# wjqkkky/TTS

Measured on AMD Instinct MI355X. Metric: mel-frames/s (Tacotron2-DDC + MB-MelGAN end-to-end), higher is better.
Workload: dtype f32; 1 GPU; C2: Tacotron2-DDC (r_init=7, r=2, sigmoid attn) + MB-MelGAN [8,4,2]x4, 32 LJ-length utterances per GPU; global_batch=32, r=2, parallelism=replicas x1

## Files before the change

### tts_amd/csrc/api_core.hip

```cpp
#include "host.h"
#include "split16.h"
#include "switches.h"

#include <cmath>
#include <cstring>
#include <memory>

static thread_local std::string g_err;
void tts_set_error(const std::string& m) { g_err = m; }

namespace ttsh {

void upload_split_rows(DevBuf& d, const std::vector<float>& w, int rows, int K) {
  bool ok = rows % 16 == 0 && K % 32 == 0 && w.size() == (size_t)rows * K;
  for (float v : w) ok &= std::fabs(v) < F16_RANGE;
  if (!ok) {
    d.reset();
    return;
  }
  d.upload(pack_split_a(rows / 16, K / 32, [&](int m, int k) { return w[(size_t)m * K + k]; }));
}

const HostT& need(const HostMap& m, const std::string& k, std::vector<int64_t> shape) {
  auto it = m.find(k);
// ... 116 lines not shown
  a.rep_pad = c.rep_pad;
  a.nphase = L.nphase;
  for (int i = 0; i < 8; ++i) a.pad_left[i] = L.pad_left[i];
  a.w_phase_stride = L.phase_stride;
  a.W = L.W.f();
  a.bias = L.bias.f();
  a.Cout = L.Cout;
  a.Cout_pad = L.Cout_pad;
  a.out = c.out;
  a.ob = c.ob;
  a.oc = c.oc;
  a.ot = c.ot;
  a.out_mul = c.out_mul;
  a.epi_act = c.epi;
  a.resid = c.resid;
  a.rb = c.rb;
  a.rc = c.rc;
  a.rt = c.rt;
  a.resid_rows = c.resid_rows;
  a.aux = c.aux;
  a.auxb = c.auxb;
  a.max_q = c.max_q;
  a.B = c.B;
  a.merged_u = c.merged_u;
  TTS_CHECK(!c.merged_u || (c.oflow && L.W16.p), "phase-merged ConvTranspose runs on split-f16 weights only");
  if (c.oflow && L.W16.p && c.nsrc == 1 && (c.s[0].sc != 1 || c.s[0].st % 4 == 0)) {
    a.W16 = L.W16.p;
    a.w16_phase_stride = L.w16_stride;
    a.oflow = c.oflow;
    launch_conv_x3(a, st);
    return;
  }
  launch_conv(a, L.tile, st);
}

void enter(tts_ctx* c, void* stream) {
  if (c->sv_live && !c->in_submit) {
    HIP_OK(hipStreamWaitEvent(c->s, c->ev_sv, 0));
    c->sv_live = false;
  }
  if (hipStreamQuery((hipStream_t)stream) == hipSuccess) return;
  (void)hipGetLastError();
  HIP_OK(hipEventRecord(c->ev_in, (hipStream_t)stream));
  HIP_OK(hipStreamWaitEvent(c->s, c->ev_in, 0));
}
void leave(tts_ctx* c, void* stream) {
// ... 150 lines not shown
```

### tts_amd/csrc/api_ge2e.hip

```cpp
#include "host.h"
#include "gsync.h"
#include "split16.h"
#include "switches.h"

#include <cmath>

using namespace ttsh;

namespace {

__global__ void pad_channels_kernel(const float* __restrict__ x, int D, int Dp, long n_rows, float* __restrict__ y) {
  for (long i = (long)blockIdx.x * blockDim.x + threadIdx.x; i < n_rows * Dp; i += (long)gridDim.x * blockDim.x) {
    const long r = i / Dp;
    const int c = (int)(i - r * Dp);
    y[i] = c < D ? x[r * D + c] : 0.f;
  }
}

__global__ __launch_bounds__(256) void ge2e_final_kernel(const float* __restrict__ src, long sb, int width,
                                                         const int* lens, int T_max, const float* __restrict__ W,
                                                         const float* __restrict__ bias, int P,
                                                         float* __restrict__ out) {
  __shared__ float v[1024], red[4];
  const int b = blockIdx.x, tid = threadIdx.x;
// ... 110 lines not shown
  TTS_CHECK(T_max >= 1 && T_max <= 100000, "speaker encoder: bad T_max");
  for (int b = 0; b < B; ++b) TTS_CHECK(h_lens[b] >= 1 && h_lens[b] <= T_max, "speaker encoder: lens out of range");
  hipStream_t s = c->s;
  const int H = G.H;
  long gen = 0;
  grow<float>(W.x, (size_t)B * T_max * G.in_pad, gen);
  grow<int>(W.lens, 64, gen);
  grow<float>(W.g, (size_t)B * T_max * 4 * H, gen);
  grow<float>(W.o, (size_t)B * T_max * H, gen);
  grow<float>(W.p, (size_t)B * T_max * G.proj, gen);
  grow<unsigned>(W.bar, BAR_WORDS, gen);
  grow<float>(W.hbuf, (size_t)2 * 64 * H, gen);
  std::vector<int> lens(h_lens, h_lens + B);
  HIP_OK(hipMemcpyAsync(W.lens.p, lens.data(), B * 4, hipMemcpyHostToDevice, s));
  pad_channels_kernel<<<1024, 256, 0, s>>>(d_x, G.in_dim, G.in_pad, (long)B * T_max, W.x.f());
  HIP_OK(hipGetLastError());
  const float* in = W.x.f();
  int din = G.in_pad;
  const bool pipe_env = sw::ge2e_pipe();
  bool piped = false;
  if (pipe_env && c->gemm_x3 && G.pipe_ok && B <= 16) {
    ConvCall cc;
    cc.lens = W.lens.i();
    cc.B = B;
    cc.oflow = x3_flag(c);
    cc.max_q = T_max;
    cc.s[0] = src_of(in, (long)T_max * din, 1, din, din, 0);
    cc.out = W.g.f();
    cc.ob = (long)T_max * 4 * H;
    cc.oc = 1;
    cc.ot = 4 * H;
    run_conv(G.gin[0], cc, s);
    const uint16_t* w16[4] = {nullptr, nullptr, nullptr, nullptr};
    const float* bias[4] = {nullptr, nullptr, nullptr, nullptr};
    for (int l = 0; l < G.nl; ++l) {
      w16[l] = l == 0 ? G.whh16[0].h() : G.wpipe[l].h();
      bias[l] = l == 0 ? nullptr : G.bpipe[l].f();
    }
    piped = launch_ge2e_pipe(w16, bias, G.nl, W.g.f(), W.lens.i(), T_max, B, W.hbuf.f(),
                             reinterpret_cast<unsigned*>(W.bar.p), W.o.f(), s);
    if (piped && G.with_proj) {
      ConvCall cp;
      cp.lens = W.lens.i();
      cp.B = B;
      cp.oflow = x3_flag(c);
      cp.max_q = T_max;
      cp.s[0] = src_of(W.o.f(), (long)T_max * H, 1, H, H, 0);
      cp.out = W.p.f();
      cp.ob = (long)T_max * G.proj;
      cp.oc = 1;
      cp.ot = G.proj;
      run_conv(G.proj_l[G.nl - 1], cp, s);
    }
  }
  for (int l = 0; l < G.nl && !piped; ++l) {
    ConvCall cc;
    cc.lens = W.lens.i();
    cc.B = B;
    cc.oflow = x3_flag(c);
    cc.max_q = T_max;
    cc.s[0] = src_of(in, (long)T_max * din, 1, din, din, 0);
    cc.out = W.g.f();
    cc.ob = (long)T_max * 4 * H;
    cc.oc = 1;
    cc.ot = 4 * H;
    run_conv(G.gin[l], cc, s);
    const bool ok = launch_lstm768_persist(W.g.f(), G.whh[l].f(), c->gemm_x3 ? G.whh16[l].h() : nullptr, W.lens.i(),
                                           T_max, B, W.hbuf.f(),
                                           reinterpret_cast<unsigned*>(W.bar.p), W.o.f(), s);
    TTS_CHECK(ok, "speaker encoder: cooperative launch unavailable");
    if (G.with_proj) {
      ConvCall cp;
      cp.lens = W.lens.i();
      cp.B = B;
      cp.oflow = x3_flag(c);
      cp.max_q = T_max;
      cp.s[0] = src_of(W.o.f(), (long)T_max * H, 1, H, H, 0);
      cp.out = W.p.f();
      cp.ob = (long)T_max * G.proj;
      cp.oc = 1;
      cp.ot = G.proj;
      run_conv(G.proj_l[l], cp, s);
      in = W.p.f();
      din = G.proj;
    } else {
      in = W.o.f();
      din = H;
    }
  }
  if (G.with_proj)
    ge2e_final_kernel<<<B, 256, 0, s>>>(W.p.f(), (long)T_max * G.proj, G.proj, W.lens.i(), T_max, nullptr, nullptr,
                                        G.proj, d_out);
  else
    ge2e_final_kernel<<<B, 256, 0, s>>>(W.o.f(), (long)T_max * H, H, W.lens.i(), T_max, G.lin_w.f(), G.lin_b.f(),
                                        G.proj, d_out);
  HIP_OK(hipGetLastError());
// ... 32 lines not shown
```

### tts_amd/csrc/api_glow.hip

```cpp
#include "host.h"

#include <cmath>
#include <cstdlib>

using namespace ttsh;

namespace {

std::pair<std::vector<float>, std::vector<float>> interleave_halves(const std::vector<float>& w,
                                                                           const std::vector<float>& b, int half,
                                                                           int rowlen) {
  std::vector<float> wo(w.size()), bo(b.size());
  for (int r = 0; r < 2 * half; ++r) {
    const int src = (r & 1) ? half + r / 2 : r / 2;
    std::copy(w.begin() + (size_t)src * rowlen, w.begin() + (size_t)(src + 1) * rowlen, wo.begin() + (size_t)r * rowlen);
    bo[r] = b[src];
  }
  return {wo, bo};
}

void glow_finalize(tts_ctx* c, int num_chars, int enc_layers, int flows, int wn_layers) {
  auto& G = c->glow;
  const auto& h = c->glow_host;
  G.ready = false;
// ... 275 lines not shown
    }
    W.h_spk.assign(h_spk, h_spk + B);
    HIP_OK(hipMemcpyAsync(W.spk.p, W.h_spk.data(), B * 4, hipMemcpyHostToDevice, s));
    launch_glow_speaker(W.spk.i(), G.emb_g.f(), G.c_in, G.c_pad, W.g.f(), B, s);
    ConvCall cc;
    cc.lens = W.ones.i();
    cc.B = B;
    cc.oflow = x3_flag(c);
    cc.max_q = 1;
    cc.s[0] = src_of(W.g.f(), G.c_pad, 1, 1, G.c_pad, 0);
    cc.out = W.gcond.f();
    cc.ob = NC;
    cc.oc = 1;
    cc.ot = 1;
    run_conv(G.cond, cc, s);
  }
  float* x = W.xa.f();
  float* x2 = W.xb.f();
  launch_glow_embed(d_ids, T, G.emb.f(), G.num_chars, H, dl, x, B, s);
  auto conv = [&](const ConvLayer& L, const float* in, int cin, float* out, int cout, int epi,
                  const float* resid = nullptr) {
    ConvCall cc;
    cc.lens = dl;
    cc.B = B;
    cc.oflow = x3_flag(c);
    cc.max_q = T;
    cc.s[0] = src_of(in, (long)cin * T, T, 1, cin, 0);
    cc.out = out;
    cc.ob = (long)cout * T;
    cc.oc = T;
    cc.ot = 1;
    cc.epi = epi;
    cc.resid = resid;
    cc.rb = (long)cout * T;
    cc.rc = T;
    cc.rt = 1;
    run_conv(L, cc, s);
  };
  if (G.tdsep || G.tfm) {
    float* h0 = W.h2.f();
    float* h1 = W.hdp.f();
    conv(G.pre_conv[0], x, H, h0, H, 0);
    launch_ln(h0, (long)H * T, H, G.pre_g[0].f(), G.pre_b[0].f(), dl, B, T, s, true);
    conv(G.pre_conv[1], h0, H, h1, H, 0);
    launch_ln(h1, (long)H * T, H, G.pre_g[1].f(), G.pre_b[1].f(), dl, B, T, s, true);
    conv(G.pre_conv[2], h1, H, h0, H, 0);
// ... 7 lines not shown
      conv(G.tfm_o[i], h0, H, x2, H, 0, x);
      launch_ln(x2, (long)H * T, H, G.tfm_g1[i].f(), G.tfm_b1[i].f(), dl, B, T, s);
      conv(G.tfm_f1[i], x2, H, big, 768, 1);
      conv(G.tfm_f2[i], big, 768, x, H, 0, x2);
      launch_ln(x, (long)H * T, H, G.tfm_g2[i].f(), G.tfm_b2[i].f(), dl, B, T, s);
    }
    for (int i = 0; i < (G.tdsep ? G.enc_layers : 0); ++i) {
      conv(G.tds_tc[i], x, H, h0, H, 6);
      launch_tds_depthwise(h0, H, T, G.tds_dw[i].f(), G.tds_dwb[i].f(), dl, h1, B, s);
      conv(G.tds_tc2[i], h1, H, x2, H, 0, x);
      std::swap(x, x2);
    }
  }
  for (int i = 0; i < (G.tdsep || G.tfm ? 0 : G.enc_layers); ++i) {
    conv(G.enc_conv[i], x, H, W.h2.f(), 2 * H, 0);
    launch_glu_ln_res(W.h2.f(), (long)2 * H * T, 2 * H, G.enc_g[i].f(), G.enc_b[i].f(), x, (long)H * T, x2,
                      (long)H * T, dl, B, T, s);
    std::swap(x, x2);
  }
  conv(G.proj_m, x, H, W.om.f(), C, 0);
  if (G.c_pad > 0) {
    ConvCall cc;
    cc.lens = dl;
    cc.B = B;
    cc.max_q = T;
    cc.nsrc = 2;
    cc.s[0] = src_of(x, (long)H * T, T, 1, H, 0);
    cc.s[1] = src_of(W.g.f(), G.c_pad, 1, 0, G.c_pad, 0);
    cc.out = W.hdp.f();
    cc.ob = (long)F * T;
    cc.oc = T;
    cc.ot = 1;
    cc.epi = 1;
    run_conv(G.dp1, cc, s);
  } else {
    conv(G.dp1, x, H, W.hdp.f(), F, 1);
  }
  launch_ln(W.hdp.f(), (long)F * T, F, G.dp_g1.f(), G.dp_b1.f(), dl, B, T, s);
  conv(G.dp2, W.hdp.f(), F, W.h2.f(), F, 1);
  launch_ln(W.h2.f(), (long)F * T, F, G.dp_g2.f(), G.dp_b2.f(), dl, B, T, s);
  conv(G.dp_proj, W.h2.f(), F, W.logw.f(), 1, 0);
  launch_glow_durations(W.logw.f(), T, dl, length_scale, W.cum.f(), W.ylens.i(), W.wceil.f(), B, s);
  HIP_OK(hipMemcpyAsync(h_ylens, W.ylens.p, B * 4, hipMemcpyDeviceToHost, s));
  HIP_OK(hipStreamSynchronize(s));
  int mx = 1;
  W.h_ylens.assign(h_ylens, h_ylens + B);
// ... 9 lines not shown
  TTS_CHECK(W.B > 0 && Ty == W.Ty, "glow: decode after encode with Ty = max(y_lengths)");
  hipStream_t s = c->s;
  const int B = W.B, Tx = W.Tx, H = G.H, C = G.C, C2 = 2 * C, K = Ty / 2;
  long gen = 0;
  const int K1 = std::max(K, 1);
  grow<float>(W.z, (size_t)B * C * Ty, gen);
  grow<float>(W.sq, (size_t)B * C2 * K1, gen);
  grow<float>(W.sq2, (size_t)B * C2 * K1, gen);
  grow<float>(W.whs, (size_t)B * 2 * H * K1, gen);
  grow<float>(W.wacts, (size_t)B * H * K1, gen);
  launch_glow_expand(W.om.f(), C, Tx, W.lens.i(), W.cum.f(), W.ylens.i(), Ty, d_noise, noise_scale, d_ymean, W.z.f(),
                     d_attn, B, s);
  HIP_OK(hipMemcpyAsync(d_logw, W.logw.p, (size_t)B * Tx * 4, hipMemcpyDeviceToDevice, s));
  HIP_OK(hipMemsetAsync(d_y, 0, (size_t)B * C * 2 * K * 4, s));
  if (K == 0) return;
  for (int b = 0; b < B; ++b) W.h_klens[b] = W.h_ylens[b] / 2;
  HIP_OK(hipMemcpyAsync(W.klens.p, W.h_klens.data(), B * 4, hipMemcpyHostToDevice, s));
  const int* kl = W.klens.i();
  launch_glow_squeeze(W.z.f(), C, Ty, W.ylens.i(), W.sq.f(), K, B, s);
  auto conv = [&](const ConvLayer& L, const float* in, int in_rows, float* out, int out_rows, const float* resid,
                  int epi, int resid_rows = 0, const float* aux = nullptr) {
    ConvCall cc;
    cc.lens = kl;
    cc.B = B;
    cc.oflow = x3_flag(c);
    cc.max_q = K;
    cc.s[0] = src_of(in, (long)in_rows * K, K, 1, L.Cin, 0);
    cc.out = out;
    cc.ob = (long)out_rows * K;
    cc.oc = K;
    cc.ot = 1;
    cc.resid = resid;
    cc.rb = (long)out_rows * K;
    cc.rc = K;
    cc.rt = 1;
    cc.epi = epi;
    cc.resid_rows = resid_rows;
    cc.aux = aux;
    cc.auxb = (long)G.flows * G.wn_layers * 2 * H;
    run_conv(L, cc, s);
  };
  float* x = W.sq.f();
  float* x2 = W.sq2.f();
  float* hid = W.whs.f();
  float* skip = W.whs.f() + (size_t)H * K;
  for (int k = G.flows - 1; k >= 0; --k) {
// ... 53 lines not shown
```

### tts_amd/csrc/api_melgan.hip

```cpp
#include "host.h"
#include "split16.h"
#include "switches.h"

#include <cmath>
#include <cstring>

using namespace ttsh;

static void melgan_finalize(tts_ctx* c, int in_ch, int out_ch, int base, const int32_t* ups, int n_up, int nres,
                     int use_pqmf) {
  auto& G = c->mg;
  const auto& m = c->mg_host;
  G.ready = false;
  TTS_CHECK(nres >= 1 && nres <= 4, "num_res_blocks must be in [1, 4] (dilation <= 27)");
  G.in_ch = in_ch;
  G.out_ch = out_ch;
  G.base = base;
  G.nres = nres;
  G.pqmf = use_pqmf;
  G.ups.assign(ups, ups + n_up);
  G.convT.clear();
  G.dconv.clear();
  G.fused.clear();
  G.convT.resize(n_up);
// ... 123 lines not shown
  int up = 1;
  for (int u : G.ups) up *= u;
  size_t maxelems = (size_t)G.base * Lb;
  {
    int mul = 1, Cc = G.base;
    for (int u : G.ups) {
      mul *= u;
      Cc /= 2;
      maxelems = std::max(maxelems, (size_t)Cc * Lb * mul);
    }
  }
  int* vld = c->vlens_override;
  if (!vld) {
    W.lens.ensure(B * 4);
    vld = W.lens.i();
  }
  W.xa.ensure((size_t)B * maxelems * 4);
  W.xb.ensure((size_t)B * maxelems * 4);
  std::vector<int> lens(h_lens, h_lens + B);
  if (!dev_lens) HIP_OK(hipMemcpyAsync(vld, lens.data(), B * 4, hipMemcpyHostToDevice, s));
  else TTS_CHECK(c->vlens_override || W.lens.bytes >= (size_t)B * 4, "vocoder lengths buffer");
  ConvCall cc;
  cc.lens = vld;
  cc.B = B;
  cc.oflow = x3_flag(c);
  cc.len_add = 2 * pad;
  if (mel_strides) {
    TTS_CHECK(mel_strides[1] >= 1 && mel_strides[2] >= 1 && mel_strides[1] < (1L << 31) && mel_strides[2] < (1L << 31) &&
                  (mel_strides[0] >= 1 || B == 1) && mel_strides[0] >= 0,
              "mel strides must be positive");
    TTS_CHECK(mel_strides[1] != 1 || (mel_strides[2] % 4 == 0 && (reinterpret_cast<uintptr_t>(mel) & 15) == 0),
              "channel stride 1 needs a frame stride divisible by 4 and a 16-byte aligned mel");
    cc.s[0] = src_of(mel, (long)mel_strides[0], (int)mel_strides[1], (int)mel_strides[2], G.in_ch, 0);
  } else {
    cc.s[0] = src_of(mel, (long)G.in_ch * M_max, M_max, 1, G.in_ch, 0);
  }
  cc.pad_mode = 1;
  cc.rep_pad = pad;
  cc.in_mul = cc.q_mul = 1;
  cc.max_q = Lb;
  float* x = W.xa.f();
  float* xo = W.xb.f();
  int C = G.base, mul = 1;
  long Ls = Lb;
  cc.out = x;
  cc.ob = (long)C * Ls;
// ... 241 lines not shown
```

### tts_amd/csrc/api_taco.hip

```cpp
#include "host.h"
#include "decoder.h"
#include "gsync.h"
#include "split16.h"
#include "switches.h"

#include <cstdio>
#include <cstring>

using namespace ttsh;

namespace {

DecDev make_dev(tts_ctx* c, int Bact) {
  auto& W = c->tws;
  DecDev d{};
  int* ci = W.ctl.i();
  d.ctl = reinterpret_cast<DecCtl*>(ci);
  d.done = ci + 4;
  d.steps = ci + 4 + BMAX;
  d.status = ci + 4 + 2 * BMAX;
  d.max_steps = ci + 4 + 3 * BMAX;
  d.lens = W.lens.i();
  d.dec_out = W.dec.f();
  d.align_out = W.align.f();
// ... 165 lines not shown
  for (int m = 0; m < MB; ++m) acc[m] = 0.f;
  for (int e = q; e < Es; e += 4) {
    const float w = WT[(long)e * N + nc];
#pragma unroll
    for (int m = 0; m < MB; ++m) {
      const float sv = m < B ? spk[m * Es + e] : 0.f;
      acc[m] = fmaf(sv, w, acc[m]);
    }
  }
  if (q > 0) {
#pragma unroll
    for (int m = 0; m < MB; ++m) red[q - 1][m][c] = acc[m];
  }
  __syncthreads();
  if (q != 0 || n >= N) return;
  const float base = n >= pj0 ? pjb[n - pj0] : 0.f;
#pragma unroll
  for (int m = 0; m < MB; ++m)
    if (m < Bp) out[(long)m * N + n] = base + (m < B ? ((acc[m] + red[0][m][c]) + red[1][m][c]) + red[2][m][c] : 0.f);
  for (int m = MB; m < Bp; ++m) out[(long)m * N + n] = base;
}

void run_encoder(tts_ctx* c, const int64_t* ids, int B, int T_max, float* enc_out, hipStream_t s,
                 const int* rowmap = nullptr) {
  auto& M = c->taco;
  auto& W = c->tws;
  const int* lens = W.lens.i();
  launch_embed_gather(ids, T_max, M.emb.f(), M.num_chars, 512, lens, B, W.x0.f(), s, rowmap);
  ConvCall cc;
  cc.lens = lens;
  cc.B = B;
  cc.oflow = x3_flag(c);
  cc.max_q = T_max;
  cc.pad_mode = 0;
  cc.epi = 1;
  cc.s[0] = src_of(W.x0.f(), (long)T_max * 512, 1, 512, 512, 0);
  cc.out = W.ca.f();
  cc.ob = (long)512 * T_max;
  cc.oc = T_max;
  cc.ot = 1;
  run_conv(M.enc[0], cc, s);
  cc.s[0] = src_of(W.ca.f(), (long)512 * T_max, T_max, 1, 512, 0);
  cc.out = W.cb.f();
  run_conv(M.enc[1], cc, s);
  cc.s[0] = src_of(W.cb.f(), (long)512 * T_max, T_max, 1, 512, 0);
  cc.out = W.ca.f();
  run_conv(M.enc[2], cc, s);
  cc.s[0] = src_of(W.ca.f(), (long)512 * T_max, T_max, 1, 512, 0);
  cc.out = W.gin.f();
  cc.ob = (long)2048 * T_max;
  cc.oc = 1;
  cc.ot = 2048;
  cc.epi = 0;
  run_conv(M.lstm_in, cc, s);
  W.enc_ndom = sw::encoder_steps()
                   ? 0
                   : launch_bilstm_persist(W.gin.f(), M.whhT.f(), c->gemm_x3 ? M.whhT16.h() : nullptr, lens, T_max, B,
                                           W.lh.f(), reinterpret_cast<unsigned*>(W.lc.p), enc_out, s);
  W.enc_persist = W.enc_ndom > 0;
  if (!W.enc_persist) {
    HIP_OK(hipMemsetAsync(enc_out, 0, (size_t)B * T_max * 512 * 4, s));
    launch_bilstm(W.gin.f(), M.whhT.f(), lens, T_max, B, W.lh.f(), W.lc.f(), enc_out, s);
  }
}

void check_encoder_barrier(tts_ctx* c) {
  if (!c->tws.enc_persist) return;
  int* pw = c->pinned + 240;
  const int nd = std::min(c->tws.enc_ndom, ENC_NDOM_MAX);
  pw[0] = pw[1] = pw[2] = pw[3] = 0;
  const unsigned* words = reinterpret_cast<const unsigned*>(c->tws.lc.p);
  for (int i = 0; i < nd; ++i) HIP_OK(hipMemcpyAsync(&pw[i], words + i * BAR_WORDS + 16, 4, hipMemcpyDeviceToHost, c->s));
  HIP_OK(hipStreamSynchronize(c->s));
  TTS_CHECK(pw[0] == 0 && pw[1] == 0 && pw[2] == 0 && pw[3] == 0, "persistent BiLSTM: grid barrier timed out (workgroups not co-resident) or preempted past TTS_BARRIER_TIMEOUT_MS; retrying the call is safe)");
}

void run_postnet(tts_ctx* c, const float* dec, long dec_b, const int* mlens, int B, int Mmax_alloc, int max_q,
                 float* out, long out_b, hipStream_t s) {
  auto& M = c->taco;
  auto& W = c->tws;
  ConvCall cc;
  cc.lens = mlens;
  cc.B = B;
  cc.oflow = x3_flag(c);
  cc.max_q = max_q;
  cc.pad_mode = 0;
  cc.epi = 2;
  cc.s[0] = src_of(dec, dec_b, 1, 80, 80, 0);
  cc.out = W.pa.f();
  cc.ob = (long)512 * Mmax_alloc;
  cc.oc = Mmax_alloc;
  cc.ot = 1;
  run_conv(M.post[0], cc, s);
  float* bufs[2] = {W.pa.f(), W.pbb.f()};
  for (int i = 1; i < 4; ++i) {
    cc.s[0] = src_of(bufs[(i - 1) & 1], (long)512 * Mmax_alloc, Mmax_alloc, 1, 512, 0);
    cc.out = bufs[i & 1];
    run_conv(M.post[i], cc, s);
  }
  cc.s[0] = src_of(bufs[1], (long)512 * Mmax_alloc, Mmax_alloc, 1, 512, 0);
  cc.out = out;
  cc.ob = out_b;
  cc.oc = 1;
  cc.ot = 80;
  cc.epi = 0;
// ... 335 lines not shown
      ta.max_steps[i] = h_max_steps[perm[i]];
    }
    taco_setup_kernel<<<1, 256, 0, s>>>(ta, W.map.i(), W.lens.i(), W.ctl.i(), fv ? x3_flag(c) : nullptr);
    HIP_OK(hipGetLastError());
  }
  int* d_map = W.map.i();
  W.thr = thr;
  TTS_CHECK(!M.variant() || use_persistent(c), "BN prenet / attention windowing / forward / Graves attention run on "
                                               "the persistent decoder only (<= 64 utterances per call on a 256-CU "
                                               "device)");
  if (M.spk_dim) {
    TTS_CHECK(d_spk_ids || d_spk_emb, "multi-speaker model: speaker ids or speaker embeddings are required");
    TTS_CHECK(use_persistent(c), "multi-speaker decoding runs on the persistent decoder only (<= 64 utterances "
                                 "per call on a 256-CU device)");
    if (d_spk_emb) {
      gather_rows<float>(d_spk_emb, W.spk.f(), d_map, M.spk_dim, B, s);
    } else {
      TTS_CHECK(M.num_spk > 0, "model has no speaker_embedding table: pass speaker embeddings");
      gather_rows<int64_t>(d_spk_ids, reinterpret_cast<int64_t*>(W.spkid.p), d_map, 1, B, s);
      launch_embed_gather(reinterpret_cast<const int64_t*>(W.spkid.p), 1, M.spk_table.f(), M.num_spk, M.spk_dim,
                          W.lens.i(), B, W.spk.f(), s);
    }
  }
  run_encoder(c, ids, B, T_max, W.enc.f(), s, d_map);
  {
    ConvCall cc;
    cc.lens = W.lens.i();
    cc.B = B;
    cc.oflow = x3_flag(c);
    cc.max_q = T_max;
    cc.s[0] = src_of(W.enc.f(), (long)T_max * 512, 1, 512, 512, 0);
    cc.out = W.penc.f();
    cc.ob = (long)T_max * 128;
    cc.oc = 1;
    cc.ot = 128;
    run_conv(M.penc, cc, s);
  }
  const int Bp = W.MT * 16;
  const bool persist = use_persistent(c);
  if (persist && !W.pslot_cal) {
    pick_barrier_blocks(reinterpret_cast<unsigned*>(W.pbar.p), PBAR_CAND, PMAX_LAUNCH, W.pslot, s);
    W.pslot_cal = true;
  }
  {
    FillList f;
    f.add(W.catt.p, (size_t)Bp * 1024 * 4);
    f.add(W.hatt.p, (size_t)Bp * 1024 * 4);
    f.add(W.hdec0.p, (size_t)Bp * 1024 * 4);
    f.add(W.hdec1.p, (size_t)Bp * 1024 * 4);
    f.add(W.cdec.p, (size_t)Bp * 1024 * 4);
// ... 29 lines not shown
    W.gr = r;
    W.gthr = thr;
  }
  for (int mt = 1; mt <= W.MT; ++mt) step_graph(c, mt, s);
  const int chunks_max = max_ms / CHUNK + 1;
  bool done = false;
  int mt = W.MT;
  for (int ch = 0; ch < chunks_max && !done; ++ch) {
    HIP_OK(hipGraphLaunch(W.graphs[mt], s));
    HIP_OK(hipMemcpyAsync(&c->pinned[2 * (ch & 1)], &reinterpret_cast<DecCtl*>(W.ctl.p)->all_done, 8,
                          hipMemcpyDeviceToHost, s));
    HIP_OK(hipEventRecord(c->ev_chunk[ch & 1], s));
    if (ch >= 1) {
      HIP_OK(hipEventSynchronize(c->ev_chunk[(ch - 1) & 1]));
      const int* pv = &c->pinned[2 * ((ch - 1) & 1)];
      if (pv[0]) done = true;
      else if (pv[1] >= 1 && pv[1] < mt) mt = pv[1];
    }
  }
  }
  taco_mlens_kernel<<<1, 64, 0, s>>>(W.ctl.i(), B, r, W.mlens.i());
  HIP_OK(hipGetLastError());
  const long fb = (long)S_cap * r * 80;
  run_postnet(c, W.dec.f(), fb, W.mlens.i(), B, S_cap * r, S_cap * r, W.post.f(), fb, s);
  gather4_rows(Gather4{{W.post.f(), W.dec.f(), W.align.f(), W.stop.f()}, {d_post, d_dec, d_align, d_stop},
                       {fb, fb, (long)S_cap * T_max, (long)S_cap}},
               d_map + BMAX, B, s);
  {
    const unsigned* lc = reinterpret_cast<const unsigned*>(W.lc.p);
    taco_status_kernel<<<1, 256, 0, s>>>(W.enc_persist ? lc : nullptr, W.enc_ndom,
                                         persist ? reinterpret_cast<const unsigned*>(W.pbar.p) : nullptr,
                                         DecSlots{{W.pslot[0], W.pslot[1], W.pslot[2], W.pslot[3]}}, c->dec_nlaunch, W.ctl.i(), c->gemm_x3 ? x3_flag(c) : nullptr, W.stat.i(),
                                         B, d_map + BMAX, r, fv ? fv->Lmin : 0, fv ? fv->vlens : nullptr);
    HIP_OK(hipGetLastError());
    int* pin = c->pinned;
    HIP_OK(hipMemcpyAsync(pin + TS_ENC, W.stat.i() + TS_ENC, (TS_N - TS_ENC) * 4, hipMemcpyDeviceToHost, s));
    if (fv) {
      HIP_OK(hipEventRecord(c->ev_status, s));
      fv->enqueue();
      HIP_OK(hipEventSynchronize(c->ev_status));
    } else {
      HIP_OK(hipStreamSynchronize(s));
    }
    TTS_CHECK(!W.enc_persist || (pin[TS_ENC] == 0 && pin[TS_ENC + 1] == 0 && pin[TS_ENC + 2] == 0 && pin[TS_ENC + 3] == 0),
              "persistent BiLSTM: grid barrier timed out (workgroups not co-resident) or preempted past "
              "TTS_BARRIER_TIMEOUT_MS; retrying the call is safe)");
    TTS_CHECK(!persist || (pin[TS_DEC] == 0 && pin[TS_DEC + 1] == 0 && pin[TS_DEC + 2] == 0 && pin[TS_DEC + 3] == 0),
// ... 39 lines not shown
  return guarded_ctx(c, [&] {
    TTS_CHECK(c && d_ids && h_lens && h_max_steps && d_dec && d_post && d_align && d_stop && h_steps && h_status,
              "null argument");
    DeviceGuard g(c->device);
    with_x3_fallback(c, [&] {
      taco_infer(c, d_ids, h_lens, B, T_max, r, h_max_steps, S_cap, thr, d_dec, d_post, d_align, d_stop, h_steps,
                 h_status, stream, d_spk_ids, d_spk_emb);
    });
  });
}

int tts_taco_encoder(tts_ctx* c, const int64_t* d_ids, const int32_t* h_lens, int B, int T_max, float* d_out,
                     void* stream) {
  return guarded_ctx(c, [&] {
    TTS_CHECK(c && d_ids && h_lens && d_out, "null argument");
    TTS_CHECK(c->taco.ready, "tacotron2 weights not finalized");
    TTS_CHECK(B >= 1 && B <= BMAX && T_max >= 1, "bad sizes");
    for (int b = 0; b < B; ++b) TTS_CHECK(h_lens[b] >= 1 && h_lens[b] <= T_max, "lens out of range");
    DeviceGuard g(c->device);
    taco_workspace(c, B, T_max, std::max(1, c->tws.S_cap), std::max(1, c->tws.r));
    enter(c, stream);
    std::vector<int> lens(h_lens, h_lens + B);
    HIP_OK(hipMemcpyAsync(c->tws.lens.p, lens.data(), B * 4, hipMemcpyHostToDevice, c->s));
    with_x3_fallback(c, [&] { run_encoder(c, d_ids, B, T_max, d_out, c->s); });
    check_encoder_barrier(c);
    leave(c, stream);
  });
}

int tts_taco_postnet(tts_ctx* c, const float* d_dec, const int32_t* h_lens, int B, int M_max, float* d_out,
                     void* stream) {
  return guarded_ctx(c, [&] {
    TTS_CHECK(c && d_dec && h_lens && d_out, "null argument");
    TTS_CHECK(c->taco.ready, "tacotron2 weights not finalized");
    TTS_CHECK(B >= 1 && B <= BMAX && M_max >= 1, "bad sizes");
    DeviceGuard g(c->device);
    auto& W = c->tws;
    long gen = W.gen;
    grow<int>(W.mlens, BMAX, gen);
    grow<float>(W.pa, (size_t)B * 512 * M_max, gen);
    grow<float>(W.pbb, (size_t)B * 512 * M_max, gen);
    W.gen = gen;
    int maxM = 0;
    for (int b = 0; b < B; ++b) {
      TTS_CHECK(h_lens[b] >= 1 && h_lens[b] <= M_max, "lens out of range");
      maxM = std::max(maxM, (int)h_lens[b]);
    }
    enter(c, stream);
    std::vector<int> lens(h_lens, h_lens + B);
    HIP_OK(hipMemcpyAsync(W.mlens.p, lens.data(), B * 4, hipMemcpyHostToDevice, c->s));
    HIP_OK(hipMemsetAsync(d_out, 0, (size_t)B * M_max * 80 * 4, c->s));
    with_x3_fallback(c, [&] {
      run_postnet(c, d_dec, (long)M_max * 80, W.mlens.i(), B, M_max, maxM, d_out, (long)M_max * 80, c->s);
    });
    HIP_OK(hipStreamSynchronize(c->s));
    leave(c, stream);
  });
}

int tts_taco_decoder_state(tts_ctx* c, int B, int T_max, float* d_att_h, float* d_att_c, float* d_dec_h,
                           float* d_dec_c, float* d_context, float* d_alpha, float* d_alpha_cum, void* stream) {
  return guarded_ctx(c, [&] {
    TTS_CHECK(c->last_B > 0, "run tts_taco_infer first");
    TTS_CHECK(B == c->last_B && T_max == c->last_T,
              "decoder state: the buffers' (B, T_max) differ from the last decode on this context");
    TTS_CHECK(c->dec_path == 1 && c->dec_nlaunch >= 1, "decoder state: the last decode did not run the persistent "
                                                       "decoder (TTS_DECODER=graph or a non-256-CU device)");
    DeviceGuard g(c->device);
    auto& W = c->tws;
    const int t_end = c->dec_end[c->dec_nlaunch - 1];
    TTS_CHECK(t_end >= 1, "decoder state: no decoder step ran");
    const float* hdec = ((t_end - 1) & 1) ? W.hdec0.f() : W.hdec1.f();
    enter(c, stream);
    taco_state_kernel<<<dim3(4, c->last_B), 256, 0, c->s>>>(W.hatt.f(), W.catt.f(), hdec, W.cdec.f(), W.ctx.f(),
                                                            W.alpha.f(), W.acum.f(), W.map.i() + BMAX, c->last_T,
                                                            c->dec_presplit ? 1 : 0, d_att_h, d_att_c, d_dec_h, d_dec_c, d_context, d_alpha,
// ... 60 lines not shown
```

### tts_amd/csrc/common.h

```cpp
#pragma once
#include <hip/hip_runtime.h>
#include <atomic>
#include <cstdint>
#include <mutex>
#include <set>
#include <string>
#include <tuple>
#include <vector>

typedef float f32x4 __attribute__((ext_vector_type(4)));

#define MFMA16(a, b, c) __builtin_amdgcn_mfma_f32_16x16x4f32((a), (b), (c), 0, 0, 0)

void tts_set_error(const std::string& msg);

#define HIP_OK(expr)                                                                   \
  do {                                                                                 \
    hipError_t _e = (expr);                                                            \
    if (_e != hipSuccess) {                                                            \
      throw std::runtime_error(std::string(#expr) + ": " + hipGetErrorString(_e));     \
    }                                                                                  \
  } while (0)

#define TTS_CHECK(cond, msg)                                                           \
// ... 63 lines not shown
  int len_add;
  int in_mul;
  int q_mul;
  int rep_pad;
  int nphase;
  int pad_left[8];
  long w_phase_stride;
  const float* W;
  const float* bias;
  int Cout, Cout_pad;
  float* out;
  long ob;
  int oc, ot;
  int out_mul;
  int epi_act;
  const float* resid;
  long rb;
  int rc, rt;
  int resid_rows;
  const float* aux;
  long auxb;
  int max_q;
  int B;
  const void* W16 = nullptr;
  long w16_phase_stride = 0;
  unsigned* oflow = nullptr;
  int merged_u = 0;
};

enum ConvTile { TILE_128x64 = 0, TILE_64x64, TILE_192x64, TILE_96x64, TILE_48x128, TILE_80x64, TILE_16x256 };
int conv_tile_tc(int tile);
int conv_tile_for_cout(int cout);
void launch_conv(const ConvArgs& a, int tile, hipStream_t s);
bool conv_x3_supported(int Cin, int Cout, int K, int dil);
void launch_conv_x3(const ConvArgs& a, hipStream_t s);
std::vector<uint16_t> pack_conv_x3(const std::vector<float>& Wm, int Cin, int Cout, int K, int nphase,
                                   long* phase_stride_bytes);
std::vector<float> merge_convT_phases(const std::vector<float>& Wm, int u, int Cin, int Cout);

void swizzle_rows16(const float* Wm, int rows, int rows_pad, int Kdim, float* dst);

struct FillList {
  static constexpr int N = 32;
  int n = 0;
  void* p[N];
  long words[N];
// ... 72 lines not shown
```

### tts_amd/csrc/conv_x3.hip

```cpp
#include "common.h"
#include "conv_epi.h"
#include "split16.h"
#include "switches.h"
#include "x3_tile.h"

#include <algorithm>
#include <mutex>
#include <map>

namespace {
constexpr int CX_XR = 80;
}

template <int MI, int NI, int WM, int WN, int KT, int RS, int SD>
__global__ __launch_bounds__(64 * WM * WN) void conv_x3_kernel(ConvArgs a, int nq, int nco, int nz) {
  constexpr int NTHR = 64 * WM * WN;
  constexpr int TC = 16 * MI * WM, TQ = 16 * NI * WN;
  constexpr int SPT = (4 * (TQ + CONV_MAX_SPAN) + NTHR - 1) / NTHR;
  static_assert(RS == KT || RS == 2 * KT, "weight ring: one or two chunks of taps");
  extern __shared__ __attribute__((aligned(16))) _Float16 shx[];

  const int ntile = nq * nco * nz;
  const int per = (ntile + 7) / 8;
  const int w = (int)(blockIdx.x % 8) * per + (int)(blockIdx.x / 8);
  if (w >= ntile) return;
  const int cot = w / (nq * nz);
  const int rem = w - cot * nq * nz;
  const int z = rem / nq;
  const int qt = rem - z * nq;

  const int ph = z % a.nphase;
  const int b = z / a.nphase;
  const int base = a.lens[b] + a.len_add;
  const int Lq = base * a.q_mul + (a.merged_u ? 1 : 0);
  const int q0 = qt * TQ;
  if (q0 >= Lq) return;
  const int co0 = cot * TC;
  const int Lin = base * a.in_mul;
  const int dil = a.dil;
  const int span = (KT - 1) * dil;
  const int ROWS = TQ + span;
  _Float16* X0 = shx;
  _Float16* X1 = shx + ROWS * CX_XR;

  const int tid = threadIdx.x;
  const int lane = tid & 63, wave = __builtin_amdgcn_readfirstlane(tid >> 6);
  const int wm = wave / WN, wn = wave % WN;
  const int nb = wn * 16 * NI + (lane & 15);
  const int kg = 8 * (lane >> 4);
  const int NCH = (a.Cin + 31) / 32;
  const int NKS = NCH * KT;
  const int mtiles = (a.Cout + 15) / 16;
  bool bad = false;

  const ConvSrc& S = a.src[0];
  const int i0 = q0 - a.pad_left[ph];
  const bool interior = (a.rep_pad == 0) && i0 >= 0 && i0 + ROWS <= Lin;
  const int rawL = a.lens[b];
  const int Lsrc = a.rep_pad ? rawL : Lin;
  const bool tmajor = S.sc == 1;
  const __amdgpu_buffer_rsrc_t xr = __builtin_amdgcn_make_buffer_rsrc(
      const_cast<float*>(S.ptr + (long)b * S.sb), 0,
      (int)min((long)0x7fffffff, ((long)(S.C - 1) * S.sc + (long)(Lsrc - 1) * S.st + 1) * 4), 0x00020000);
  int voff[SPT], sgv[SPT], srow[SPT];
  bool sval[SPT];
#pragma unroll
  for (int j = 0; j < SPT; ++j) {
    const int e = tid + NTHR * j;
    const int g = e / ROWS;
    srow[j] = e - g * ROWS;
    sgv[j] = g;
    int i = i0 + srow[j];
    bool valid = true;
    if (!interior) {
      i = map_pad_index(i, Lin, a.pad_mode, valid);
      if (a.rep_pad) i -= a.rep_pad;
    }
    i = i < 0 ? 0 : (i >= Lsrc ? Lsrc - 1 : i);
    sval[j] = valid && g < 4;
    voff[j] = (min(g, 3) * 8 * S.sc + i * S.st) * 4;
  }
// ... 193 lines not shown
    conv_epilogue<MI, NI, WN>(a, acc, b, ph, q0, co0, wm, wn, lane);
  }
  if (bad) __hip_atomic_fetch_or(a.oflow, 1u, __ATOMIC_RELAXED, __HIP_MEMORY_SCOPE_AGENT);
}

enum { CX_T128 = 0, CX_T192, CX_T96, CX_T64, CX_T80, CX_T48, CX_NONE };

static int cx_tile(int Cout) {
  if (Cout % 128 == 0) return CX_T128;
  if (Cout == 192) return CX_T192;
  if (Cout == 96) return CX_T96;
  if (Cout == 80) return CX_T80;
  if (Cout == 48) return CX_T48;
  if (Cout % 64 == 0) return CX_T64;
  if (Cout % 80 == 0) return CX_T80;
  return CX_NONE;
}

bool conv_x3_supported(int Cin, int Cout, int K, int dil) {
  return Cin % 8 == 0 && Cin >= 8 && cx_tile(Cout) != CX_NONE && (K == 1 || K == 2 || K == 3 || K == 5 || K == 7) &&
         (K - 1) * dil <= CONV_MAX_SPAN;
}

template <int MI, int NI, int WM, int WN, int KT, int RS, int SD>
static void cx_launch(const ConvArgs& a, hipStream_t s) {
  constexpr int TC = 16 * MI * WM, TQ = 16 * NI * WN;
  ensure_dyn_lds((const void*)conv_x3_kernel<MI, NI, WM, WN, KT, RS, SD>, 160 * 1024);
  const int nq = (a.max_q + TQ - 1) / TQ, nco = (a.Cout + TC - 1) / TC, nz = a.B * a.nphase;
  const long ntile = (long)nq * nco * nz;
  TTS_CHECK(ntile < (1L << 30), "conv_x3: grid too large");
  const int per = (int)((ntile + 7) / 8);
  const size_t lds = (size_t)2 * (TQ + (KT - 1) * a.dil) * CX_XR * 2;
  conv_x3_kernel<MI, NI, WM, WN, KT, RS, SD><<<dim3(8 * per), 64 * WM * WN, lds, s>>>(a, nq, nco, nz);
}

template <int MI, int NI, int WM, int WN, int KT, int RS, int SD>
static long cx_cost_k(const ConvArgs& a) {
  constexpr int TC = 16 * MI * WM, TQ = 16 * NI * WN;
  const void* f = (const void*)conv_x3_kernel<MI, NI, WM, WN, KT, RS, SD>;
  const size_t lds = (size_t)2 * (TQ + (KT - 1) * a.dil) * CX_XR * 2;
  static std::mutex mu;
  static std::map<size_t, long> slots_by_lds;
  long slots;
  ensure_dyn_lds(f, 160 * 1024);
  const int cus = device_cu_count();
  {
    std::lock_guard<std::mutex> lk(mu);
    auto it = slots_by_lds.find(lds);
    if (it == slots_by_lds.end()) {
      int nb = 0;
      HIP_OK(hipOccupancyMaxActiveBlocksPerMultiprocessor(&nb, f, 64 * WM * WN, lds));
      it = slots_by_lds.emplace(lds, std::max(1L, (long)nb * cus)).first;
    }
    slots = it->second;
  }
  const long tiles = (long)((a.max_q + TQ - 1) / TQ) * ((a.Cout + TC - 1) / TC) * a.B * a.nphase;
  return (tiles + slots - 1) / slots * TQ;
}
template <int MI, int NI, int WM, int WN, int SD12>
static long cx_cost(const ConvArgs& a) {
  switch (a.K) {
    case 1: return cx_cost_k<MI, NI, WM, WN, 1, 2, SD12>(a);
    case 2: return cx_cost_k<MI, NI, WM, WN, 2, 2 * SD12, SD12>(a);
    case 3: return cx_cost_k<MI, NI, WM, WN, 3, 3, 1>(a);
    case 5: return cx_cost_k<MI, NI, WM, WN, 5, 5, 2>(a);
    case 7: return cx_cost_k<MI, NI, WM, WN, 7, 7, 1>(a);
    default: return 0;
  }
}

template <int MI, int NI, int WM, int WN, int SD12>
static void cx_taps(const ConvArgs& a, hipStream_t s) {
  switch (a.K) {
    case 1: cx_launch<MI, NI, WM, WN, 1, 2, SD12>(a, s); break;
    case 2: cx_launch<MI, NI, WM, WN, 2, 2 * SD12, SD12>(a, s); break;
    case 3: cx_launch<MI, NI, WM, WN, 3, 3, 1>(a, s); break;
    case 5: cx_launch<MI, NI, WM, WN, 5, 5, 2>(a, s); break;
    case 7: cx_launch<MI, NI, WM, WN, 7, 7, 1>(a, s); break;
    default: TTS_CHECK(false, "conv_x3: unsupported tap count");
// ... 58 lines not shown
```

### tts_amd/csrc/host.h

```cpp
#pragma once
#include "common.h"
#include "launch.h"
#include "../../include/ttship.h"

#include <algorithm>
#include <functional>
#include <map>
#include <mutex>
#include <stdexcept>
#include <string>
#include <vector>

namespace ttsh {

constexpr int CHUNK = 8;
constexpr int BMAX = 64;

struct DevBuf {
  void* p = nullptr;
  size_t bytes = 0;
  DevBuf() = default;
  DevBuf(const DevBuf&) = delete;
  DevBuf& operator=(const DevBuf&) = delete;
  DevBuf(DevBuf&& o) noexcept : p(o.p), bytes(o.bytes) { o.p = nullptr; o.bytes = 0; }
// ... 50 lines not shown
};

void pack_conv(ConvLayer& L, const std::vector<float>& Wm, const std::vector<float>& bias, int Cin, int Cout,
               int K, int dil, int nphase, const int* pad_left);
void pack_conv_x3_only(ConvLayer& L, const std::vector<float>& Wm, const std::vector<float>& bias, int Cin, int Cout,
                       int K);

struct ConvCall {
  ConvSrc s[2];
  int nsrc = 1;
  int pad_mode = 0;
  const int* lens = nullptr;
  int len_add = 0, in_mul = 1, q_mul = 1, rep_pad = 0, out_mul = 1;
  float* out = nullptr;
  long ob = 0;
  int oc = 0, ot = 0;
  int epi = 0;
  const float* resid = nullptr;
  long rb = 0;
  int rc = 0, rt = 0, resid_rows = 0;
  const float* aux = nullptr;
  long auxb = 0;
  int max_q = 0, B = 0;
  unsigned* oflow = nullptr;
  int merged_u = 0;
};

void run_conv(const ConvLayer& L, const ConvCall& c, hipStream_t st);

inline ConvSrc src_of(const float* p, long sb, int sc, int st, int C, int act) { return ConvSrc{p, sb, sc, st, C, act}; }

std::vector<float> lstm_tile_rows(const std::vector<float>& W, int H, int K);
std::vector<float> hcat(const std::vector<std::pair<const float*, int>>& parts, int rows);
std::vector<float> slice_cols(const std::vector<float>& W, int rows, int K, int c0, int c1);
std::vector<float> swz(const std::vector<float>& Wm, int rows, int K);
void fold_convbn(const HostMap& m, const std::string& pfx, int Cin, int Cout, int K, std::vector<float>& Wm,
                 std::vector<float>& bias);

struct TacoModel {
  bool ready = false;
  int num_chars = 0, r_init = 7, softmax = 0;
  DevBuf emb;
  ConvLayer enc[3], lstm_in, penc, post[5];
  DevBuf whhT;
  DevBuf whhT16;
  DevBuf pre1, pre2, att_p, att_pre, att_bias, dec_w, dec_bias, WqT, Wloc, Wdense, v, proj_w, proj_b;
// ... 333 lines not shown
```

### tts_amd/csrc/x3_tile.h

```cpp
#pragma once
#include "common.h"
#include "split16.h"

__device__ __forceinline__ __amdgpu_buffer_rsrc_t x3_rsrc(const void* p) {
  return __builtin_amdgcn_make_buffer_rsrc(const_cast<void*>(p), 0, 0x7fffffff, 0x00020000);
}

__device__ __forceinline__ void x3_load_a(h8 (&r)[2], __amdgpu_buffer_rsrc_t w, int wlo, int blk) {
  r[0] = __builtin_bit_cast(h8, __builtin_amdgcn_raw_buffer_load_b128(w, wlo, blk, 0));
  r[1] = __builtin_bit_cast(h8, __builtin_amdgcn_raw_buffer_load_b128(w, wlo + 16, blk, 0));
}

struct X3Tile {
  int b, q0, L;
};
template <int TQ>
__device__ __forceinline__ void x3_tile_scan(int* tcum, int* tlen, int lane, int L) {
  const int n = (L + TQ - 1) / TQ;
  int v = n;
#pragma unroll
  for (int o = 1; o < 64; o <<= 1) {
    const int y = __shfl_up(v, o, 64);
    if (lane >= o) v += y;
  }
  tcum[lane] = v - n;
  tlen[lane] = L;
  if (lane == 63) tcum[64] = v;
}
template <int TQ>
__device__ __forceinline__ X3Tile x3_tile_of(const int* tcum, const int* tlen, int B, int lane, int i) {
  const bool hit = lane < B && tcum[lane] <= i && i < tcum[lane + 1];
  const unsigned long long m = __ballot(hit);
  const int b = __builtin_amdgcn_readfirstlane(m ? __ffsll((long long)m) - 1 : 0);
  X3Tile r;
  r.b = b;
  r.q0 = __builtin_amdgcn_readfirstlane((i - tcum[b]) * TQ);
  r.L = __builtin_amdgcn_readfirstlane(tlen[b]);
  return r;
}

inline long x3_tile_count(const int* h_lens, int B, int len_add, int mul, int TQ, const char* who) {
  long ntiles = 0;
  for (int b = 0; b < B; ++b) ntiles += ((long)(h_lens[b] + len_add) * mul + TQ - 1) / TQ;
  TTS_CHECK(ntiles < (1L << 30), std::string(who) + ": too many tiles");
  return ntiles;
}
```

Before: 1.311 million mel-frames/s.

## Compact conv_x3 grid to per-row tile counts using host-side lengths

Result: no change. 1.321 million mel-frames/s, median of 6 (+0.8%).

```diff
diff --git a/tts_amd/csrc/api_core.hip b/tts_amd/csrc/api_core.hip
--- a/tts_amd/csrc/api_core.hip
+++ b/tts_amd/csrc/api_core.hip
@@ -162,6 +162,7 @@
   a.auxb = c.auxb;
   a.max_q = c.max_q;
   a.B = c.B;
+  a.h_lens = c.h_lens;
   a.merged_u = c.merged_u;
   TTS_CHECK(!c.merged_u || (c.oflow && L.W16.p), "phase-merged ConvTranspose runs on split-f16 weights only");
   if (c.oflow && L.W16.p && c.nsrc == 1 && (c.s[0].sc != 1 || c.s[0].st % 4 == 0)) {
diff --git a/tts_amd/csrc/api_ge2e.hip b/tts_amd/csrc/api_ge2e.hip
--- a/tts_amd/csrc/api_ge2e.hip
+++ b/tts_amd/csrc/api_ge2e.hip
@@ -156,6 +156,7 @@
   if (pipe_env && c->gemm_x3 && G.pipe_ok && B <= 16) {
     ConvCall cc;
     cc.lens = W.lens.i();
+    cc.h_lens = lens.data();
     cc.B = B;
     cc.oflow = x3_flag(c);
     cc.max_q = T_max;
@@ -176,6 +177,7 @@
     if (piped && G.with_proj) {
       ConvCall cp;
       cp.lens = W.lens.i();
+      cp.h_lens = lens.data();
       cp.B = B;
       cp.oflow = x3_flag(c);
       cp.max_q = T_max;
@@ -190,6 +192,7 @@
   for (int l = 0; l < G.nl && !piped; ++l) {
     ConvCall cc;
     cc.lens = W.lens.i();
+    cc.h_lens = lens.data();
     cc.B = B;
     cc.oflow = x3_flag(c);
     cc.max_q = T_max;
@@ -206,6 +209,7 @@
     if (G.with_proj) {
       ConvCall cp;
       cp.lens = W.lens.i();
+      cp.h_lens = lens.data();
       cp.B = B;
       cp.oflow = x3_flag(c);
       cp.max_q = T_max;
diff --git a/tts_amd/csrc/api_glow.hip b/tts_amd/csrc/api_glow.hip
--- a/tts_amd/csrc/api_glow.hip
+++ b/tts_amd/csrc/api_glow.hip
@@ -321,6 +321,7 @@
                   const float* resid = nullptr) {
     ConvCall cc;
     cc.lens = dl;
+    cc.h_lens = lens.data();
     cc.B = B;
     cc.oflow = x3_flag(c);
     cc.max_q = T;
@@ -374,6 +375,7 @@
   if (G.c_pad > 0) {
     ConvCall cc;
     cc.lens = dl;
+    cc.h_lens = lens.data();
     cc.B = B;
     cc.max_q = T;
     cc.nsrc = 2;
@@ -429,6 +431,7 @@
                   int epi, int resid_rows = 0, const float* aux = nullptr) {
     ConvCall cc;
     cc.lens = kl;
+    cc.h_lens = W.h_klens.data();
     cc.B = B;
     cc.oflow = x3_flag(c);
     cc.max_q = K;
diff --git a/tts_amd/csrc/api_melgan.hip b/tts_amd/csrc/api_melgan.hip
--- a/tts_amd/csrc/api_melgan.hip
+++ b/tts_amd/csrc/api_melgan.hip
@@ -169,6 +169,7 @@
   else TTS_CHECK(c->vlens_override || W.lens.bytes >= (size_t)B * 4, "vocoder lengths buffer");
   ConvCall cc;
   cc.lens = vld;
+  cc.h_lens = lens.data();
   cc.B = B;
   cc.oflow = x3_flag(c);
   cc.len_add = 2 * pad;
diff --git a/tts_amd/csrc/api_taco.hip b/tts_amd/csrc/api_taco.hip
--- a/tts_amd/csrc/api_taco.hip
+++ b/tts_amd/csrc/api_taco.hip
@@ -211,13 +211,14 @@
 }
 
 void run_encoder(tts_ctx* c, const int64_t* ids, int B, int T_max, float* enc_out, hipStream_t s,
-                 const int* rowmap = nullptr) {
+                 const int* rowmap = nullptr, const int* h_lens = nullptr) {
   auto& M = c->taco;
   auto& W = c->tws;
   const int* lens = W.lens.i();
   launch_embed_gather(ids, T_max, M.emb.f(), M.num_chars, 512, lens, B, W.x0.f(), s, rowmap);
   ConvCall cc;
   cc.lens = lens;
+  cc.h_lens = h_lens;
   cc.B = B;
   cc.oflow = x3_flag(c);
   cc.max_q = T_max;
@@ -264,12 +265,13 @@
   TTS_CHECK(pw[0] == 0 && pw[1] == 0 && pw[2] == 0 && pw[3] == 0, "persistent BiLSTM: grid barrier timed out (workgroups not co-resident) or preempted past TTS_BARRIER_TIMEOUT_MS; retrying the call is safe)");
 }
 
-void run_postnet(tts_ctx* c, const float* dec, long dec_b, const int* mlens, int B, int Mmax_alloc, int max_q,
-                 float* out, long out_b, hipStream_t s) {
+void run_postnet(tts_ctx* c, const float* dec, long dec_b, const int* mlens, const int* h_mlens, int B,
+                 int Mmax_alloc, int max_q, float* out, long out_b, hipStream_t s) {
   auto& M = c->taco;
   auto& W = c->tws;
   ConvCall cc;
   cc.lens = mlens;
+  cc.h_lens = h_mlens;
   cc.B = B;
   cc.oflow = x3_flag(c);
   cc.max_q = max_q;
@@ -651,10 +653,13 @@
                           W.lens.i(), B, W.spk.f(), s);
     }
   }
-  run_encoder(c, ids, B, T_max, W.enc.f(), s, d_map);
+  std::vector<int> tlens(B);
+  for (int i = 0; i < B; ++i) tlens[i] = h_lens[perm[i]];
+  run_encoder(c, ids, B, T_max, W.enc.f(), s, d_map, tlens.data());
   {
     ConvCall cc;
     cc.lens = W.lens.i();
+    cc.h_lens = tlens.data();
     cc.B = B;
     cc.oflow = x3_flag(c);
     cc.max_q = T_max;
@@ -730,7 +735,9 @@
   taco_mlens_kernel<<<1, 64, 0, s>>>(W.ctl.i(), B, r, W.mlens.i());
   HIP_OK(hipGetLastError());
   const long fb = (long)S_cap * r * 80;
-  run_postnet(c, W.dec.f(), fb, W.mlens.i(), B, S_cap * r, S_cap * r, W.post.f(), fb, s);
+  std::vector<int> mbound(B);
+  for (int i = 0; i < B; ++i) mbound[i] = h_max_steps[perm[i]] * r;
+  run_postnet(c, W.dec.f(), fb, W.mlens.i(), mbound.data(), B, S_cap * r, S_cap * r, W.post.f(), fb, s);
   gather4_rows(Gather4{{W.post.f(), W.dec.f(), W.align.f(), W.stop.f()}, {d_post, d_dec, d_align, d_stop},
                        {fb, fb, (long)S_cap * T_max, (long)S_cap}},
                d_map + BMAX, B, s);
@@ -816,7 +823,7 @@
     enter(c, stream);
     std::vector<int> lens(h_lens, h_lens + B);
     HIP_OK(hipMemcpyAsync(c->tws.lens.p, lens.data(), B * 4, hipMemcpyHostToDevice, c->s));
-    with_x3_fallback(c, [&] { run_encoder(c, d_ids, B, T_max, d_out, c->s); });
+    with_x3_fallback(c, [&] { run_encoder(c, d_ids, B, T_max, d_out, c->s, nullptr, lens.data()); });
     check_encoder_barrier(c);
     leave(c, stream);
   });
@@ -845,7 +852,8 @@
     HIP_OK(hipMemcpyAsync(W.mlens.p, lens.data(), B * 4, hipMemcpyHostToDevice, c->s));
     HIP_OK(hipMemsetAsync(d_out, 0, (size_t)B * M_max * 80 * 4, c->s));
     with_x3_fallback(c, [&] {
-      run_postnet(c, d_dec, (long)M_max * 80, W.mlens.i(), B, M_max, maxM, d_out, (long)M_max * 80, c->s);
+      run_postnet(c, d_dec, (long)M_max * 80, W.mlens.i(), lens.data(), B, M_max, maxM, d_out, (long)M_max * 80,
+                  c->s);
     });
     HIP_OK(hipStreamSynchronize(c->s));
     leave(c, stream);
diff --git a/tts_amd/csrc/common.h b/tts_amd/csrc/common.h
--- a/tts_amd/csrc/common.h
+++ b/tts_amd/csrc/common.h
@@ -109,6 +109,7 @@
   long auxb;
   int max_q;
   int B;
+  const int* h_lens = nullptr;
   const void* W16 = nullptr;
   long w16_phase_stride = 0;
   unsigned* oflow = nullptr;
diff --git a/tts_amd/csrc/conv_x3.hip b/tts_amd/csrc/conv_x3.hip
--- a/tts_amd/csrc/conv_x3.hip
+++ b/tts_amd/csrc/conv_x3.hip
@@ -12,26 +12,55 @@
 constexpr int CX_XR = 80;
 }
 
+template <int TQ>
+__device__ __forceinline__ void cx_scan_rows(const ConvArgs& a, int& lraw, int& n, int& v) {
+  const int ln = threadIdx.x & 63;
+  lraw = ln < a.B ? a.lens[ln] : 0;
+  n = ln < a.B ? x3_row_tiles((lraw + a.len_add) * a.q_mul + (a.merged_u ? 1 : 0), a.max_q, TQ) : 0;
+  v = n;
+#pragma unroll
+  for (int o = 1; o < 64; o <<= 1) {
+    const int y = __shfl_up(v, o, 64);
+    if (ln >= o) v += y;
+  }
+}
+__device__ __forceinline__ bool cx_deal_tile(int p, int nco, int lraw, int n, int v, int& cot, int& z, int& qt, int& lb) {
+  int t;
+  if (!x3_deal(p, __builtin_amdgcn_readlane(v, 63), nco, &cot, &t)) return false;
+  const unsigned long long m = __ballot(x3_row_holds(v, n, t));
+  if (!m) return false;
+  z = __builtin_amdgcn_readfirstlane(__ffsll((long long)m) - 1);
+  qt = t - __builtin_amdgcn_readfirstlane(__shfl(v - n, z, 64));
+  lb = __builtin_amdgcn_readfirstlane(__shfl(lraw, z, 64));
+  return true;
+}
+
 template <int MI, int NI, int WM, int WN, int KT, int RS, int SD>
-__global__ __launch_bounds__(64 * WM * WN) void conv_x3_kernel(ConvArgs a, int nq, int nco, int nz) {
+__global__ __launch_bounds__(64 * WM * WN) void conv_x3_kernel(ConvArgs a, int nq, int nco, int nz, int compact) {
   constexpr int NTHR = 64 * WM * WN;
   constexpr int TC = 16 * MI * WM, TQ = 16 * NI * WN;
   constexpr int SPT = (4 * (TQ + CONV_MAX_SPAN) + NTHR - 1) / NTHR;
   static_assert(RS == KT || RS == 2 * KT, "weight ring: one or two chunks of taps");
   extern __shared__ __attribute__((aligned(16))) _Float16 shx[];
-
-  const int ntile = nq * nco * nz;
-  const int per = (ntile + 7) / 8;
-  const int w = (int)(blockIdx.x % 8) * per + (int)(blockIdx.x / 8);
-  if (w >= ntile) return;
-  const int cot = w / (nq * nz);
-  const int rem = w - cot * nq * nz;
-  const int z = rem / nq;
-  const int qt = rem - z * nq;
-
+  int cot, z, qt, lb;
+  if (compact) {
+    int lraw, n, v;
+    cx_scan_rows<TQ>(a, lraw, n, v);
+    if (!cx_deal_tile((int)blockIdx.x, nco, lraw, n, v, cot, z, qt, lb)) return;
+  } else {
+    const int ntile = nq * nco * nz;
+    const int per = (ntile + 7) / 8;
+    const int w = (int)(blockIdx.x % 8) * per + (int)(blockIdx.x / 8);
+    if (w >= ntile) return;
+    cot = w / (nq * nz);
+    const int rem = w - cot * nq * nz;
+    z = rem / nq;
+    qt = rem - z * nq;
+    lb = a.lens[z / a.nphase];
+  }
   const int ph = z % a.nphase;
   const int b = z / a.nphase;
-  const int base = a.lens[b] + a.len_add;
+  const int base = lb + a.len_add;
   const int Lq = base * a.q_mul + (a.merged_u ? 1 : 0);
   const int q0 = qt * TQ;
   if (q0 >= Lq) return;
@@ -56,7 +85,7 @@
   const ConvSrc& S = a.src[0];
   const int i0 = q0 - a.pad_left[ph];
   const bool interior = (a.rep_pad == 0) && i0 >= 0 && i0 + ROWS <= Lin;
-  const int rawL = a.lens[b];
+  const int rawL = lb;
   const int Lsrc = a.rep_pad ? rawL : Lin;
   const bool tmajor = S.sc == 1;
   const __amdgpu_buffer_rsrc_t xr = __builtin_amdgcn_make_buffer_rsrc(
@@ -296,16 +325,22 @@
          (K - 1) * dil <= CONV_MAX_SPAN;
 }
 
+static bool cx_compact(const ConvArgs& a) { return a.B <= 64 && a.nphase == 1; }
+static long cx_row_tiles(const ConvArgs& a, int TQ) {
+  return x3_deal_rows(a.h_lens, a.B, a.len_add, a.q_mul, a.merged_u ? 1 : 0, a.max_q, TQ);
+}
+
 template <int MI, int NI, int WM, int WN, int KT, int RS, int SD>
 static void cx_launch(const ConvArgs& a, hipStream_t s) {
   constexpr int TC = 16 * MI * WM, TQ = 16 * NI * WN;
   ensure_dyn_lds((const void*)conv_x3_kernel<MI, NI, WM, WN, KT, RS, SD>, 160 * 1024);
   const int nq = (a.max_q + TQ - 1) / TQ, nco = (a.Cout + TC - 1) / TC, nz = a.B * a.nphase;
-  const long ntile = (long)nq * nco * nz;
-  TTS_CHECK(ntile < (1L << 30), "conv_x3: grid too large");
-  const int per = (int)((ntile + 7) / 8);
+  const bool compact = cx_compact(a);
+  const long grid = x3_deal_grid(compact ? cx_row_tiles(a, TQ) : (long)nq * nz, nco);
+  TTS_CHECK(grid < (1L << 30), "conv_x3: grid too large");
+  if (grid == 0) return;
   const size_t lds = (size_t)2 * (TQ + (KT - 1) * a.dil) * CX_XR * 2;
-  conv_x3_kernel<MI, NI, WM, WN, KT, RS, SD><<<dim3(8 * per), 64 * WM * WN, lds, s>>>(a, nq, nco, nz);
+  conv_x3_kernel<MI, NI, WM, WN, KT, RS, SD><<<dim3((unsigned)grid), 64 * WM * WN, lds, s>>>(a, nq, nco, nz, compact);
 }
 
 template <int MI, int NI, int WM, int WN, int KT, int RS, int SD>
@@ -328,7 +363,12 @@
     }
     slots = it->second;
   }
-  const long tiles = (long)((a.max_q + TQ - 1) / TQ) * ((a.Cout + TC - 1) / TC) * a.B * a.nphase;
+  const long nco = (a.Cout + TC - 1) / TC;
+  if (cx_compact(a)) {
+    const long per = (cx_row_tiles(a, TQ) * nco + 7) / 8, xslots = std::max(1L, slots / 8);
+    return (per + xslots - 1) / xslots * TQ;
+  }
+  const long tiles = (long)((a.max_q + TQ - 1) / TQ) * nco * a.B * a.nphase;
   return (tiles + slots - 1) / slots * TQ;
 }
 template <int MI, int NI, int WM, int WN, int SD12>
diff --git a/tts_amd/csrc/host.h b/tts_amd/csrc/host.h
--- a/tts_amd/csrc/host.h
+++ b/tts_amd/csrc/host.h
@@ -96,6 +96,7 @@
   const float* aux = nullptr;
   long auxb = 0;
   int max_q = 0, B = 0;
+  const int* h_lens = nullptr;
   unsigned* oflow = nullptr;
   int merged_u = 0;
 };
diff --git a/tts_amd/csrc/x3_tile.h b/tts_amd/csrc/x3_tile.h
--- a/tts_amd/csrc/x3_tile.h
+++ b/tts_amd/csrc/x3_tile.h
@@ -1,4 +1,36 @@
 #pragma once
+
+#ifdef __HIPCC__
+#define X3_HD __host__ __device__ __forceinline__
+#else
+#define X3_HD inline
+#endif
+X3_HD int x3_row_tiles(int L, int max_q, int TQ) {
+  const int n = L > 0 ? (L + TQ - 1) / TQ : 0, cap = (max_q + TQ - 1) / TQ;
+  return n < cap ? n : cap;
+}
+X3_HD bool x3_deal(int p, int T, int nco, int* cot, int* t) {
+  const long long real = (long long)T * nco;
+  const int x = p % 8, j = p / 8;
+  const int w0 = (int)(x * real / 8), w1 = (int)((x + 1) * real / 8);
+  if (j >= w1 - w0) return false;
+  const int w = w0 + j;
+  *cot = w / T;
+  *t = w - *cot * T;
+  return true;
+}
+X3_HD bool x3_row_holds(int incl, int n, int t) { return incl - n <= t && t < incl; }
+inline long x3_deal_rows(const int* h_lens, int B, int len_add, int q_mul, int extra, int max_q, int TQ) {
+  long T = 0;
+  for (int b = 0; b < B; ++b) {
+    const long L = h_lens ? ((long)h_lens[b] + len_add) * q_mul + extra : max_q;
+    T += x3_row_tiles((int)(L < max_q ? L : max_q), max_q, TQ);
+  }
+  return T;
+}
+inline long x3_deal_grid(long T_host, int nco) { return 8 * ((T_host * nco + 7) / 8); }
+
+#ifdef __HIPCC__
 #include "common.h"
 #include "split16.h"
 
@@ -45,3 +77,4 @@
   TTS_CHECK(ntiles < (1L << 30), std::string(who) + ": too many tiles");
   return ntiles;
 }
+#endif
```
